# noveens/reviews4rec

Hardware: AMD Instinct MI355X
Metric: train ratings/sec (higher is better)
Workload: dtype f32

## Files before the change

### include/r4r.h

```cpp
#ifndef R4R_H
#define R4R_H

#include <stddef.h>
#include <stdint.h>

#ifdef __cplusplus
extern "C" {
#endif

#define R4R_OK 0
#define R4R_ERR_ARG (-1)
#define R4R_ERR_LAUNCH (-2)
#define R4R_ERR_WORKSPACE (-3)

int r4r_version(void);
const char *r4r_last_error(void);

size_t r4r_textcnn_ws_bytes(int64_t N, int T, int E, int F, int64_t V);
int r4r_textcnn_fwd(const float *table, int64_t V, const int64_t *idx,
                    const float *conv_w, const float *conv_b,
                    float *pooled, int32_t *argmax,
                    void *ws, size_t ws_bytes,
                    int64_t N, int T, int E, int F, void *stream);

// ... 67 lines not shown
int r4r_sqdist_mean_fwd(const float *a, const float *b, float *out, int64_t N, int L, void *stream);
int r4r_sqdist_mean_bwd(const float *a, const float *b, const float *g_out, float *g_a, float *g_b,
                        int64_t N, int L, void *stream);

int r4r_adam_chunk_elems(void);
int r4r_adam_multi(int ntensor, const uint64_t *p, const uint64_t *g, const uint64_t *m, const uint64_t *v,
                   const int64_t *numel, float lr, double beta1, double beta2, float eps,
                   float weight_decay, int64_t step, const int64_t *step_dev, void *stream);
int r4r_adam_gathered(float *p, const float *gathered, int world, float *g_sum, float *m, float *v,
                      int64_t numel, float lr, double beta1, double beta2, float eps,
                      float weight_decay, int64_t step, void *stream);
int r4r_adam_gathered_guarded(float *p, const float *gathered, int world, float *g_sum, float *m, float *v,
                              int64_t numel, float lr, double beta1, double beta2, float eps,
                              float weight_decay, int64_t step, const uint32_t *abort_word, void *stream);

int r4r_peer_segment_create(int64_t bytes, void **ptr, uint8_t *handle);
int r4r_peer_segment_open(const uint8_t *handle, void **ptr);
int r4r_peer_segment_close(void *ptr);
int r4r_peer_segment_destroy(void *ptr);
int r4r_peer_push(const float *src, int64_t numel, const uint64_t *peer_dst, const uint64_t *peer_flags,
                  uint32_t *arrive, int rank, int world, uint32_t epoch, const uint32_t *wait_flags,
                  uint32_t *timed_out, double timeout_s, void *stream);
int r4r_peer_wait(const uint32_t *flags, int world, uint32_t epoch, uint32_t *timed_out, double timeout_s, void *stream);


#define R4R_CONV_AUTO 0
#define R4R_CONV_DIRECT 1
#define R4R_CONV_PROJECT 2
int r4r_deepconn_nparam(void);
int r4r_deepconn_layout(int E, int L, int64_t *offsets, int64_t *sizes, int64_t *total);
size_t r4r_deepconn_ws_bytes(int64_t B, int T, int E, int L, int64_t V);
size_t r4r_deepconn_ws_mult_offset(int64_t B, int T, int E, int L, int64_t V);
size_t r4r_deepconn_ws_count_offset(int64_t B, int T, int E, int L, int64_t V, int tower, int buffer);
int r4r_deepconn_step(const float *table, int64_t V, const int64_t *user_idx, const int64_t *item_idx,
                      const float *y, float *flat_p, float *flat_g,
                      float *pred, float *se, float *sse_accum,
                      void *ws, size_t ws_bytes,
                      int64_t B, int T, int E, int L,
                      float dropout_p, int training, uint64_t seed, uint64_t offset,
                      float inv_denom, int conv_algo, int token_buffer, int tokens_ready,
                      const int64_t *next_user_idx, const int64_t *next_item_idx,
                      float *flat_m, float *flat_v, float lr, double beta1, double beta2, float eps,
                      float weight_decay, int64_t adam_step, void *stream);
int r4r_deepconn_tokens(const int64_t *user_idx, const int64_t *item_idx, void *ws, size_t ws_bytes,
                        int64_t B, int T, int E, int L, int64_t V, int conv_algo, int token_buffer,
                        int discard, void *stream);

#define R4R_TIMING_TEXTCNN_FWD 0
#define R4R_TIMING_TEXTCNN_WGRAD 1
#define R4R_TIMING_ADAM 2
#define R4R_TIMING_PROJ_GEMM 3
#define R4R_TIMING_PROJ_GATHER 4
#define R4R_TIMING_SLOTS 8
int r4r_timing_enable(int slot_mask);
int r4r_timing_read(int slot, double *total_ms, int64_t *count, int reset);

size_t r4r_mf_ws_bytes(int64_t B, int D, int64_t n_users, int64_t n_items);
size_t r4r_mf_ws_persist_bytes(int64_t B, int D, int64_t n_users, int64_t n_items);
size_t r4r_mf_ws_mult_offset(int64_t B, int D, int64_t n_users, int64_t n_items);
size_t r4r_mf_ws_grad_offset(int64_t B, int D, int64_t n_users, int64_t n_items, int which);
int r4r_mf_step(const int64_t *uid, const int64_t *iid, const float *y,
                const uint64_t *p, const uint64_t *m, const uint64_t *v,
                int64_t n_users, int64_t n_items, int D,
                float *pred, float *se, float *sse_accum, void *ws, size_t ws_bytes, int64_t B,
                float dropout_p, int training, uint64_t seed, uint64_t offset, float inv_denom,
                int sweep_period, int64_t sweep_base, int sweep_all,
                float lr, double beta1, double beta2, float eps, float weight_decay, int64_t adam_step,
                void *stream);

int r4r_mf_rows_flush(const uint64_t *p, const uint64_t *m, const uint64_t *v,
                      int64_t n_users, int64_t n_items, int D, void *ws, size_t ws_bytes, int64_t B,
                      int sweep_period, int64_t sweep_base,
                      float lr, double beta1, double beta2, float eps, float weight_decay, int64_t adam_step,
                      void *stream);
size_t r4r_mf_ws_flag_offset(int64_t B, int D, int64_t n_users, int64_t n_items);

// ... 337 lines not shown
```

### reviews4rec_amd/csrc/common.h

```cpp
#pragma once
#include <hip/hip_runtime.h>
#include <hip/hip_ext.h>
#include <stdint.h>
#include <stdio.h>

#include "../../include/r4r.h"

namespace r4r {

void set_error(const char *fmt, ...);

bool timing_on();
void timing_begin(int id, hipStream_t st, void **token);
void timing_begin(int id, hipStream_t st, void **token, bool chain);
void timing_end(void *token, hipStream_t st);

bool timing_kernel_events(int id, hipEvent_t *start, hipEvent_t *stop);

struct ScopedTiming {
    void *tok = nullptr;
    hipStream_t st;
    ScopedTiming(int id, hipStream_t s, bool chain = false) : st(s) { if (timing_on()) timing_begin(id, s, &tok, chain); }
    ~ScopedTiming() { if (tok) timing_end(tok, st); }
};
// ... 55 lines not shown
__device__ __forceinline__ void wave_lds_fence() {
    __builtin_amdgcn_fence(__ATOMIC_RELEASE, "wavefront");
    __builtin_amdgcn_wave_barrier();
    __builtin_amdgcn_fence(__ATOMIC_ACQUIRE, "wavefront");
}

__device__ __forceinline__ uint32_t philox_first_word(uint64_t ctr, uint64_t seed) {
    uint32_t c0 = (uint32_t)ctr, c1 = (uint32_t)(ctr >> 32), c2 = 0u, c3 = 0u;
    uint32_t k0 = (uint32_t)seed, k1 = (uint32_t)(seed >> 32);
#pragma unroll
    for (int r = 0; r < 10; ++r) {
        const uint64_t p0 = (uint64_t)0xD2511F53u * c0;
        const uint64_t p1 = (uint64_t)0xCD9E8D57u * c2;
        const uint32_t n0 = (uint32_t)(p1 >> 32) ^ c1 ^ k0;
        const uint32_t n1 = (uint32_t)p1;
        const uint32_t n2 = (uint32_t)(p0 >> 32) ^ c3 ^ k1;
        const uint32_t n3 = (uint32_t)p0;
        c0 = n0; c1 = n1; c2 = n2; c3 = n3;
        k0 += 0x9E3779B9u; k1 += 0xBB67AE85u;
    }
    return c0;
}

inline int64_t cdiv(int64_t a, int64_t b) { return (a + b - 1) / b; }

template <class T>
__device__ __forceinline__ const T &kernel_args() {
    typedef const T __attribute__((address_space(4))) *kernarg_ptr;
    kernarg_ptr p = (kernarg_ptr)__builtin_amdgcn_kernarg_segment_ptr();
    asm volatile("" : "+s"(p));
    return *(const T *)p;
}


}
```

### reviews4rec_amd/csrc/engine.hip

```cpp
#include <stdlib.h>

#include "trace_device.h"
#include "textcnn.h"
#include "wgrad_device.h"
#include "tokens_device.h"
#include "adam_device.h"

namespace r4r {

constexpr int F_CONV = 100;
constexpr int FM_K = 8;
constexpr int MAX_L = 128;

enum { P_UCW = 0, P_UCB, P_UFW, P_UFB, P_ICW, P_ICB, P_IFW, P_IFB, P_FMV, P_FMLW, P_FMLB, P_GB, P_COUNT };

struct Layout {
    int64_t off[P_COUNT], size[P_COUNT], total;
};

static Layout make_layout(int E, int L) {
    Layout lay;
    const int64_t sz[P_COUNT] = {(int64_t)F_CONV * 3 * E, F_CONV, (int64_t)L * F_CONV, L,
                                 (int64_t)F_CONV * 3 * E, F_CONV, (int64_t)L * F_CONV, L,
                                 (int64_t)2 * L * FM_K, 2 * L, 1, 1};
    int64_t o = 0;
    for (int i = 0; i < P_COUNT; ++i) {
        lay.off[i] = o;
        lay.size[i] = sz[i];
        o += (sz[i] + 31) & ~(int64_t)31;
    }
    lay.total = o;
    return lay;
}

struct HeadArgs {
    const float *pmax[2]; const int *parg[2];
    const float *fc_w[2]; const float *fc_b[2];
    const float *V, *lin_w, *lin_b, *gbias;
    const float *y;
    float *pooled[2]; int *argmax[2];
    float *g_pooled[2];
    float *mult;
    float *x, *s, *g, *gz;
    float *pred, *se;
    int64_t B;
    int L, tiles, training, want_grad;
    float p_drop, inv_denom;
    uint64_t seed, offset;
};


constexpr int HEAD_MAX_TILES = 8;

#define SEL2(arr, s) ((s) ? (arr)[1] : (arr)[0])
HEAD_TRACE_DEFINE(r4r_debug_dc_head_trace)
template <int ML>
__global__ __launch_bounds__(256) void deepconn_head_wg_kernel(HeadArgs a) {
    HEAD_STAMP(0)
    constexpr int N2 = 2 * ML, PARTS = 256 / N2;
    __shared__ float sw[2][ML][F_CONV + 1];
    __shared__ float sfb[N2], slw[N2], sz[N2];
    __shared__ float sV[N2][FM_K];
    __shared__ float sp[2][F_CONV + 4];
    __shared__ float red[N2][PARTS + 1];
    const int tid = threadIdx.x, lane = tid & 63, w = tid >> 6;
    const int64_t b = blockIdx.x;
    const int L = a.L, n = 2 * L;
    const float lin_b0 = a.lin_b[0], gbias0 = a.gbias[0], yb = a.y ? a.y[b] : 0.f;

    constexpr int FQ = F_CONV / 4;
    typedef float hq4 __attribute__((ext_vector_type(4)));
    constexpr int WREGS = (2 * ML * FQ + 255) / 256;
    hq4 wreg[WREGS];
    const int wtot = 2 * L * FQ;
#pragma unroll
    for (int k = 0; k < WREGS; ++k) {
        const int i = min(tid + 256 * k, wtot - 1);
        const int t = i >= L * FQ;
        wreg[k] = *reinterpret_cast<const hq4 *>(SEL2(a.fc_w, t) + 4 * (i - t * L * FQ));
    }
    const int tn = min(tid, n - 1);
    const float fbreg = SEL2(a.fc_b, tn >= L)[tn - (tn >= L ? L : 0)];
    const float lwreg = a.lin_w[tn];
    constexpr int VREGS = (N2 * FM_K + 255) / 256;
    float vreg[VREGS];
#pragma unroll
    for (int k = 0; k < VREGS; ++k) vreg[k] = a.V[min(tid + 256 * k, n * FM_K - 1)];

    {
        const int t = w >> 1, f = lane + 64 * (w & 1), fc = min(f, F_CONV - 1);
// ... 131 lines not shown
                    float sv = 0.f;
#pragma unroll
                    for (int k = 0; k < FM_K; ++k) if (lane == k) sv = sk_keep[k];
                    a.s[b * FM_K + lane] = sv;
                }
                if (lane == 0) a.g[b] = g;
            }
        }
    }
    if (!want) return;
    __syncthreads();
    HEAD_STAMP(3)
    if (tid < 2 * F_CONV) {
        const int t = tid >= F_CONV, f = tid - t * F_CONV;
        float acc = 0.f;
        for (int l = 0; l < L; ++l) acc = fmaf(sz[t * L + l], sw[t][l][f], acc);
        SEL2(a.g_pooled, t)[b * F_CONV + f] = acc;
    }
    HEAD_STAMP(4)
}

struct HeadGradArgs {
    const float *pooled[2];
    const float *x, *s, *g, *gz;
    const float *V;
    const float *se;
    float *g_fc_w[2], *g_fc_b[2], *g_V, *g_lin_w, *g_lin_b, *g_gb;
    float *sse_accum;
    int64_t B;
    int L;
};

constexpr int HG_ROWS = 16, HG_COLS = 16;
__device__ __forceinline__ void head_grad_block(const HeadGradArgs &a, int blk) {
    __shared__ float red[HG_ROWS][HG_COLS];
    const int ox = threadIdx.x & (HG_COLS - 1), rg = threadIdx.x / HG_COLS;
    const int L = a.L, n = 2 * L;
    const int n_fcw = L * F_CONV;
    const int seg[9] = {n_fcw, L, n_fcw, L, n * FM_K, n, 1, 1, 1};
    int o = blk * HG_COLS + ox;
    int which = -1, local = 0, acc_o = o;
#pragma unroll
    for (int k = 0; k < 9; ++k) {
        if (which < 0) {
            if (acc_o < seg[k]) { which = k; local = acc_o; }
            else acc_o -= seg[k];
        }
    }
    float s = 0.f;
    if (which >= 0) {
        const bool is_w = which == 0 || which == 2, is_b = which == 1 || which == 3, is_v = which == 4, is_lw = which == 5;
        const int t = which >> 1;
        const int wl = local / F_CONV, wf = local - wl * F_CONV;
        const int vi = local / FM_K, vk = local - vi * FM_K;
        const float *pa = (is_w || is_b) ? a.gz : (which == 8 ? a.se : a.g);
        const int64_t sa = (is_w || is_b) ? n : 1;
        const int64_t oa = is_w ? t * L + wl : (is_b ? t * L + local : 0);
        const bool useb = is_w || is_v, usec = is_v || is_lw;
        const float *pb = is_w ? a.pooled[t & 1] : (is_v ? a.s : a.g);
        const int64_t sb = is_w ? F_CONV : (is_v ? FM_K : 1), ob = is_w ? wf : (is_v ? vk : 0);
        const float *pc = usec ? a.x : a.g;
        const int64_t sc = usec ? n : 1, oc = is_v ? vi : (is_lw ? local : 0);
        const float cv = is_v ? a.V[local] : 0.f;
        constexpr int HB = 8;
        for (int64_t b0 = rg; b0 < a.B; b0 += (int64_t)HG_ROWS * HB) {
            float va[HB], vb[HB], vc[HB];
#pragma unroll
            for (int k = 0; k < HB; ++k) {
                const int64_t b = min(b0 + (int64_t)k * HG_ROWS, a.B - 1);
                va[k] = pa[b * sa + oa];
                vb[k] = pb[b * sb + ob];
                vc[k] = pc[b * sc + oc];
            }
#pragma unroll
            for (int k = 0; k < HB; ++k) {
                const float B_ = useb ? vb[k] : 1.f, C_ = usec ? vc[k] : 1.f;
                const float term = va[k] * (B_ * C_ - C_ * C_ * cv);
                if (b0 + (int64_t)k * HG_ROWS < a.B) s += term;
            }
        }
    }
    red[rg][ox] = s;
    __syncthreads();
    if (rg == 0 && which >= 0) {
        float t = 0.f;
#pragma unroll
        for (int r = 0; r < HG_ROWS; ++r) t += red[r][ox];
        switch (which) {
            case 0: a.g_fc_w[0][local] = t; break;
            case 1: a.g_fc_b[0][local] = t; break;
            case 2: a.g_fc_w[1][local] = t; break;
            case 3: a.g_fc_b[1][local] = t; break;
            case 4: a.g_V[local] = t; break;
            case 5: a.g_lin_w[local] = t; break;
            case 6: a.g_lin_b[0] = t; break;
            case 7: a.g_gb[0] = t; break;
            default: if (a.sse_accum) a.sse_accum[0] += t; break;
        }
    }
}

BWD_TRACE_DEFINE(r4r_debug_dc_bwd_trace)
struct DcBackwardArgs {
    WgradArgs w;
    HeadGradArgs h;
    int hg_blocks;
    TokenArgs nx;
};
__global__ __launch_bounds__(WG_THREADS, 8) void deepconn_backward_kernel(DcBackwardArgs) {
    const DcBackwardArgs &A = kernel_args<DcBackwardArgs>();
    const WgradArgs &w = A.w;
    const HeadGradArgs &h = A.h;
    const TokenArgs &nx = A.nx;
    const int hg_blocks = A.hg_blocks;
    BWD_STAMP(0, wall_clock64())
    BWD_STAMP(2, (unsigned long long)blockIdx.z + 1)
    if (blockIdx.z == 1 || blockIdx.z == 2) {
        wgrad_block(w, blockIdx.x, blockIdx.y, blockIdx.z - 1);
    } else if (blockIdx.z == 0) {
        for (int blk = blockIdx.y * gridDim.x + blockIdx.x; blk < hg_blocks; blk += gridDim.x * gridDim.y) {
            head_grad_block(h, blk);
            __syncthreads();
        }
    } else {
        token_mark_block(nx, blockIdx.y * gridDim.x + blockIdx.x, gridDim.x * gridDim.y, WG_THREADS);
    }
#ifdef R4R_TRACE
    __syncthreads();
#endif
    BWD_STAMP(1, wall_clock64())
}

constexpr int RED_THREADS = 256;
struct FusedAdam {
    float *p, *m, *v;
    const float *g;
    int64_t lo[2], hi[2];
    AdamScalars s;
    int on;
};
__global__ __launch_bounds__(RED_THREADS) void deepconn_reduce_kernel(WgradArgs w, int red_blocks, int comp_blocks,
                                                                      TokenArgs nx, FusedAdam opt) {
    const int bx = blockIdx.x;
    if (bx < red_blocks) {
        const WgradTower &tw = w.t[blockIdx.y];
        const int nw = w.F * 3 * w.E;
        const int i = bx * RED_THREADS + threadIdx.x;
        const float *gp0 = i < nw ? tw.d_w + i : (i < nw + w.F ? tw.d_b + (i - nw) : nullptr);
        const int64_t o = gp0 ? gp0 - opt.g : 0;
        float P = 0.f, M = 0.f, V = 0.f;
        if (opt.on && gp0) { P = opt.p[o]; M = opt.m[o]; V = opt.v[o]; }
        float *dst;
        const float g = wgrad_reduce_elem(w, blockIdx.y, i, dst);
        if (opt.on && dst) {
            adam_elem(P, g, M, V, opt.s);
            opt.p[o] = P; opt.m[o] = M; opt.v[o] = V;
        }
    } else if (bx < red_blocks + comp_blocks) {
        token_compact_auto<RED_THREADS / 64>(nx.t[blockIdx.y], nx.V, bx - red_blocks);
    } else {
        const int64_t o = opt.lo[blockIdx.y] + (int64_t)(bx - red_blocks - comp_blocks) * RED_THREADS + threadIdx.x;
        if (o < opt.hi[blockIdx.y]) {
            float P = opt.p[o], M = opt.m[o], V = opt.v[o];
            adam_elem(P, opt.g[o], M, V, opt.s);
            opt.p[o] = P; opt.m[o] = M; opt.v[o] = V;
        }
    }
}

__global__ void sse_only_kernel(const float *__restrict__ se, float *__restrict__ accum, int64_t B) {
    __shared__ float red[256];
    float s = 0.f;
    for (int64_t i = threadIdx.x; i < B; i += 256) s += se[i];
    red[threadIdx.x] = s;
    __syncthreads();
    for (int off = 128; off > 0; off >>= 1) {
        if ((int)threadIdx.x < off) red[threadIdx.x] += red[threadIdx.x + off];
        __syncthreads();
    }
    if (threadIdx.x == 0) accum[0] += red[0];
}

struct StepWs {
    float *wp[2], *pmax[2]; int *parg[2];
    int *flags[2][2], *slot[2][2], *list[2][2], *count[2][2]; float *ptab[2];
    float *pooled[2]; int *argmax[2]; float *g_pooled[2];
    float *mult, *x, *s, *g, *gz;
    float *part_w[2], *part_b[2];
    size_t bytes;
};

static StepWs carve(void *ws, int64_t B, int T, int E, int L, int64_t V) {
    StepWs w;
    char *p = static_cast<char *>(ws);
    auto take = [&](size_t nbytes) { char *r = p; p += align256(nbytes); return r; };
    const size_t tiles128 = (size_t)(T + 2 + 127) / 128;
    const int ns = textcnn_wgrad_splits(B);
    for (int t = 0; t < 2; ++t) {
        w.wp[t] = reinterpret_cast<float *>(take(textcnn_wp_floats(E) * 4));
        w.pmax[t] = reinterpret_cast<float *>(take((size_t)B * tiles128 * NP * 4));
        w.parg[t] = reinterpret_cast<int *>(take((size_t)B * tiles128 * NP * 4));
        w.pooled[t] = reinterpret_cast<float *>(take((size_t)B * F_CONV * 4));
// ... 17 lines not shown
    w.bytes = (size_t)(p - static_cast<char *>(ws));
    return w;
}

}

using namespace r4r;

extern "C" int r4r_deepconn_nparam(void) { return P_COUNT; }

extern "C" int r4r_deepconn_layout(int E, int L, int64_t *offsets, int64_t *sizes, int64_t *total) {
    R4R_REQUIRE(E > 0 && L > 0 && L <= MAX_L && offsets && sizes && total, "deepconn_layout: bad arguments");
    const Layout lay = make_layout(E, L);
    for (int i = 0; i < P_COUNT; ++i) { offsets[i] = lay.off[i]; sizes[i] = lay.size[i]; }
    *total = lay.total;
    return R4R_OK;
}

extern "C" size_t r4r_deepconn_ws_bytes(int64_t B, int T, int E, int L, int64_t V) {
    if (B < 0 || T <= 0 || E <= 0 || L <= 0 || V <= 0) return 0;
    return carve(nullptr, B, T, E, L, V).bytes;
}

extern "C" size_t r4r_deepconn_ws_mult_offset(int64_t B, int T, int E, int L, int64_t V) {
    char base[1];
    const StepWs w = carve(base, B, T, E, L, V);
    return (size_t)(reinterpret_cast<char *>(w.mult) - base);
}

extern "C" size_t r4r_deepconn_ws_count_offset(int64_t B, int T, int E, int L, int64_t V, int tower, int buffer) {
    char base[1];
    const StepWs w = carve(base, B, T, E, L, V);
    return (size_t)(reinterpret_cast<char *>(w.count[buffer & 1][tower & 1]) - base);
}

extern "C" int r4r_deepconn_tokens(const int64_t *user_idx, const int64_t *item_idx, void *ws, size_t ws_bytes,
                                   int64_t B, int T, int E, int L, int64_t V, int conv_algo, int token_buffer,
                                   int discard, void *stream) {
    R4R_REQUIRE(user_idx && item_idx && ws, "deepconn_tokens: null pointer");
    R4R_REQUIRE(token_buffer == 0 || token_buffer == 1, "deepconn_tokens: token_buffer must be 0 or 1");
    if (ws_bytes < r4r_deepconn_ws_bytes(B, T, E, L, V)) {
        set_error("deepconn_tokens: workspace %zu < %zu bytes", ws_bytes, r4r_deepconn_ws_bytes(B, T, E, L, V));
        return R4R_ERR_WORKSPACE;
    }
    if (B == 0 || textcnn_pick_algo(conv_algo, B, T, E, F_CONV) != R4R_CONV_PROJECT) return R4R_OK;
    const StepWs w = carve(ws, B, T, E, L, V);
    if (discard) {
        for (int t = 0; t < 2; ++t) (void)hipMemsetAsync(w.count[token_buffer][t], 0, sizeof(int), as_stream(stream));
        return check_launch("deepconn_tokens(discard)");
    }
    ProjTower pt[2];
    const int64_t *idx[2] = {user_idx, item_idx};
    for (int t = 0; t < 2; ++t) {
        pt[t] = ProjTower{};
        pt[t].idx = idx[t];
        pt[t].flags = w.flags[token_buffer][t]; pt[t].slot = w.slot[token_buffer][t];
        pt[t].list = w.list[token_buffer][t]; pt[t].count = w.count[token_buffer][t];
    }
    return textcnn_proj_tokens_launch(V, pt, 2, B, T, false, as_stream(stream));
}

extern "C" int r4r_deepconn_step(const float *table, int64_t V, const int64_t *user_idx, const int64_t *item_idx,
                                 const float *y, float *flat_p, float *flat_g,
                                 float *pred, float *se, float *sse_accum,
                                 void *ws, size_t ws_bytes,
                                 int64_t B, int T, int E, int L,
// ... 43 lines not shown
            pt[t].conv_w = P[t ? P_ICW : P_UCW];
            pt[t].conv_b = P[t ? P_ICB : P_UCB];
            pt[t].flags = w.flags[token_buffer][t]; pt[t].slot = w.slot[token_buffer][t];
            pt[t].list = w.list[token_buffer][t]; pt[t].count = w.count[token_buffer][t];
            pt[t].ptab = w.ptab[t]; pt[t].pmax = w.pmax[t]; pt[t].parg = w.parg[t]; pt[t].wimg = w.wp[t];
        }
        if (!tokens_ready)
            if (int rc = textcnn_proj_tokens_launch(V, pt, 2, B, T, false, st)) return rc;
        if (int rc = textcnn_proj_compute_launch(table, V, pt, 2, B, T, E, F_CONV, st)) return rc;
        tiles = proj_tiles(T);
    } else {
        FwdTower ft[2];
        for (int t = 0; t < 2; ++t) {
            ft[t].idx = idx[t];
            ft[t].conv_w = P[t ? P_ICW : P_UCW];
            ft[t].conv_b = P[t ? P_ICB : P_UCB];
            ft[t].wp = w.wp[t]; ft[t].pmax = w.pmax[t]; ft[t].parg = w.parg[t];
        }
        if (int rc = textcnn_fwd_launch(table, ft, 2, B, T, E, F_CONV, st)) return rc;
        tiles = textcnn_tiles(T);
    }

    HeadArgs h;
    for (int t = 0; t < 2; ++t) {
        h.pmax[t] = w.pmax[t]; h.parg[t] = w.parg[t];
        h.fc_w[t] = P[t ? P_IFW : P_UFW]; h.fc_b[t] = P[t ? P_IFB : P_UFB];
        h.pooled[t] = w.pooled[t]; h.argmax[t] = w.argmax[t]; h.g_pooled[t] = w.g_pooled[t];
    }
    h.V = P[P_FMV]; h.lin_w = P[P_FMLW]; h.lin_b = P[P_FMLB]; h.gbias = P[P_GB];
    h.y = y; h.mult = w.mult; h.x = w.x; h.s = w.s; h.g = w.g; h.gz = w.gz;
    h.pred = pred; h.se = se;
    h.B = B; h.L = L; h.tiles = tiles; h.training = training; h.want_grad = flat_g != nullptr;
    h.p_drop = dropout_p; h.inv_denom = inv_denom; h.seed = seed; h.offset = offset;
    if (L <= 16) deepconn_head_wg_kernel<16><<<(unsigned)B, 256, 0, st>>>(h);
    else if (L <= 32) deepconn_head_wg_kernel<32><<<(unsigned)B, 256, 0, st>>>(h);
    else if (L <= 64) deepconn_head_wg_kernel<64><<<(unsigned)B, 256, 0, st>>>(h);
    else deepconn_head_wg_kernel<128><<<(unsigned)B, 256, 0, st>>>(h);

    if (!flat_g) {
        if (y && sse_accum) sse_only_kernel<<<1, 256, 0, st>>>(se, sse_accum, B);
        return check_launch("deepconn_step(forward)");
    }

    HeadGradArgs hg;
    for (int t = 0; t < 2; ++t) {
        hg.pooled[t] = w.pooled[t];
        hg.g_fc_w[t] = G[t ? P_IFW : P_UFW]; hg.g_fc_b[t] = G[t ? P_IFB : P_UFB];
    }
    hg.x = w.x; hg.s = w.s; hg.g = w.g; hg.gz = w.gz; hg.V = P[P_FMV]; hg.se = se;
    hg.g_V = G[P_FMV]; hg.g_lin_w = G[P_FMLW]; hg.g_lin_b = G[P_FMLB]; hg.g_gb = G[P_GB];
    hg.sse_accum = sse_accum; hg.B = B; hg.L = L;
    const int nout = 2 * (L * F_CONV + L) + 2 * L * FM_K + 2 * L + 3;
    const int hg_blocks = (nout + HG_COLS - 1) / HG_COLS;

    WgradTower wt[2];
    WgradArgs wa;
    for (int t = 0; t < 2; ++t) {
        wt[t].idx = idx[t]; wt[t].g_pooled = w.g_pooled[t]; wt[t].argmax = w.argmax[t];
        wt[t].part_w = w.part_w[t]; wt[t].part_b = w.part_b[t];
        wt[t].d_w = G[t ? P_ICW : P_UCW]; wt[t].d_b = G[t ? P_ICB : P_UCB];
    }
    for (int k = 0; k < MAX_TOWERS; ++k) wa.t[k] = wt[k < 2 ? k : 0];
    wa.table = table; wa.N = B; wa.T = T; wa.E = E; wa.F = F_CONV;
    wa.table_bytes = (int64_t)V * E * 4;
    wa.nsplit = textcnn_wgrad_splits(B);
    wa.per_split = (int)cdiv(B, wa.nsplit);
    const bool prefetch = next_user_idx && algo == R4R_CONV_PROJECT;
    TokenArgs nx{};
    if (prefetch) {
        ProjTower nt[2];
        const int64_t *nidx[2] = {next_user_idx, next_item_idx};
        const int ob = token_buffer ^ 1;
        for (int t = 0; t < 2; ++t) {
            nt[t] = ProjTower{};
            nt[t].idx = nidx[t];
            nt[t].flags = w.flags[ob][t]; nt[t].slot = w.slot[ob][t];
            nt[t].list = w.list[ob][t]; nt[t].count = w.count[ob][t];
        }
        nx = make_token_args(V, nt, 2, B, T);
    }
    {
        ScopedTiming tm(R4R_TIMING_TEXTCNN_WGRAD, st);
        deepconn_backward_kernel<<<dim3(F_CONV, wa.nsplit, prefetch ? 4 : 3), WG_THREADS, 0, st>>>(DcBackwardArgs{wa, hg, hg_blocks, nx});
    }
    const int red_blocks = (F_CONV * 3 * E + F_CONV + RED_THREADS - 1) / RED_THREADS;
    const int comp_blocks = prefetch ? (int)cdiv((V + 3) / 4, RED_THREADS * compact_groups(V)) : 0;
    FusedAdam opt{};
    int opt_blocks = 0;
    if (flat_m) {
        opt.on = 1;
        opt.p = flat_p; opt.m = flat_m; opt.v = flat_v; opt.g = flat_g;
        opt.lo[0] = lay.off[P_UFW]; opt.hi[0] = lay.off[P_ICW];
        opt.lo[1] = lay.off[P_IFW]; opt.hi[1] = lay.total;
        opt.s = adam_make_scalars(lr, beta1, beta2, eps, weight_decay, adam_step, nullptr);
        const int64_t longest = opt.hi[0] - opt.lo[0] > opt.hi[1] - opt.lo[1] ? opt.hi[0] - opt.lo[0] : opt.hi[1] - opt.lo[1];
        opt_blocks = (int)cdiv(longest, RED_THREADS);
    }
    deepconn_reduce_kernel<<<dim3(red_blocks + comp_blocks + opt_blocks, 2), RED_THREADS, 0, st>>>(
        wa, red_blocks, comp_blocks, nx, opt);
    return check_launch("deepconn_step");
}

extern "C" int r4r_sse_accumulate(const float *se, int64_t n, float *accum, void *stream) {
    R4R_REQUIRE(accum && (se || n == 0) && n >= 0, "sse_accumulate: bad arguments");
    if (n == 0) return R4R_OK;
    sse_only_kernel<<<1, 256, 0, as_stream(stream)>>>(se, accum, n);
    return check_launch("sse_accumulate");
}
```

### reviews4rec_amd/csrc/wgrad_device.h

```cpp
#pragma once
#include "textcnn.h"

namespace r4r {

typedef float wg_f32x4 __attribute__((ext_vector_type(4)));

constexpr int WG_THREADS = 256;

struct WgradArgs {
    WgradTower t[MAX_TOWERS];
    const float *table;
    int64_t N;
    int T, E, F, per_split, nsplit;
    int64_t table_bytes = 0;
};

constexpr int WG_CHUNK = 16;
constexpr int WG_FLIGHT = 8;

template <bool FIRST>
__device__ __forceinline__ void wgrad_block_pass(const WgradArgs &a, int f, int s, int tower, int v0,
                                                 long (&s_off)[WG_CHUNK][3], float (&s_g)[WG_CHUNK]) {
    const WgradTower &tw = a.t[tower];
    const float *__restrict__ table = a.table;
    const int64_t *__restrict__ idx = tw.idx;
    const float *__restrict__ gp = tw.g_pooled;
    const int *__restrict__ argmax = tw.argmax;
    const int T = a.T, E = a.E, F = a.F;
    const int64_t n0 = (int64_t)s * a.per_split;
    const int64_t n1 = min(a.N, n0 + (int64_t)a.per_split);
    const int nvec = 3 * E / 4;
    const int tid = threadIdx.x;
    wg_f32x4 acc[2] = {(wg_f32x4){0.f, 0.f, 0.f, 0.f}, (wg_f32x4){0.f, 0.f, 0.f, 0.f}};
    int vj[2], ve[2];
#pragma unroll
    for (int k = 0; k < 2; ++k) {
        const int v = v0 + tid + k * WG_THREADS;
        vj[k] = (v * 4) / E;
        ve[k] = v * 4 - vj[k] * E;
    }
    float sb = 0.f;
    const bool buf_ok = a.table_bytes > 0 && a.table_bytes < (1ll << 32);
    const __amdgpu_buffer_rsrc_t rsrc = __builtin_amdgcn_make_buffer_rsrc(const_cast<float *>(table), 0, buf_ok ? (int)(unsigned)a.table_bytes : 0, 0x00020000);
    for (int64_t c0 = n0; c0 < n1; c0 += WG_CHUNK) {
        const int nd = (int)min((int64_t)WG_CHUNK, n1 - c0);
        __syncthreads();
        if (tid < nd * 3) {
            const int d = tid / 3, j = tid - d * 3;
            const int64_t n = c0 + d;
            const int p = argmax[n * F + f];
// ... 28 lines not shown
                        }
                    }
                }
            }
        } else {
#pragma unroll
            for (int k = 0; k < 2; ++k) {
                if (v0 + tid + k * WG_THREADS < nvec) {
#pragma unroll 4
                    for (int d = 0; d < nd; ++d) {
                        const long off = s_off[d][vj[k]];
                        if (off >= 0) acc[k] += s_g[d] * *reinterpret_cast<const wg_f32x4 *>(table + off + ve[k]);
                    }
                }
            }
        }
        if (FIRST && tid == 0)
            for (int d = 0; d < nd; ++d) sb += s_g[d];
    }
#pragma unroll
    for (int k = 0; k < 2; ++k) {
        const int v = v0 + tid + k * WG_THREADS;
        if (v < nvec) *reinterpret_cast<wg_f32x4 *>(tw.part_w + ((size_t)s * F + f) * 3 * E + v * 4) = acc[k];
    }
    if (FIRST && tid == 0) tw.part_b[(size_t)s * F + f] = sb;
}

__device__ __forceinline__ void wgrad_block(const WgradArgs &a, int f, int s, int tower) {
    __shared__ long s_off[WG_CHUNK][3];
    __shared__ float s_g[WG_CHUNK];
    wgrad_block_pass<true>(a, f, s, tower, 0, s_off, s_g);
    const int nvec = 3 * a.E / 4;
    for (int v0 = 2 * WG_THREADS; v0 < nvec; v0 += 2 * WG_THREADS) wgrad_block_pass<false>(a, f, s, tower, v0, s_off, s_g);
}


constexpr int WG_SUPER = 96;
static_assert(WG_SUPER % WG_CHUNK == 0, "whole streaming rounds per resolved super-chunk");
__device__ __forceinline__ void wgrad_block_packed(const WgradArgs &a, int fgroup, int s, int tower) {
    __shared__ long p_off[4][WG_SUPER][3];
    __shared__ float p_g[4][WG_SUPER];
    const WgradTower &tw = a.t[tower];
    const float *__restrict__ table = a.table;
    const int64_t *__restrict__ idx = tw.idx;
    const float *__restrict__ gp = tw.g_pooled;
    const int *__restrict__ argmax = tw.argmax;
    const int T = a.T, E = a.E, F = a.F;
    const int64_t n0 = (int64_t)s * a.per_split;
    const int64_t n1 = min(a.N, n0 + (int64_t)a.per_split);
    const int nvec = 3 * E / 4;
    const int wave = threadIdx.x >> 6, lane = threadIdx.x & 63;
    const int f = fgroup * 4 + wave;
    const bool live = f < F;
    wg_f32x4 acc = (wg_f32x4){0.f, 0.f, 0.f, 0.f};
    const int vj = (lane * 4) / E, ve = lane * 4 - vj * E;
    float sb = 0.f;
    constexpr int NRES = (WG_SUPER * 3 + 63) / 64;
    for (int64_t c0 = n0; c0 < n1; c0 += WG_SUPER) {
        const int nd = (int)min((int64_t)WG_SUPER, n1 - c0);
        __syncthreads();
        if (live) {
            int pv[NRES];
            float gv[NRES];
#pragma unroll
            for (int k = 0; k < NRES; ++k) {
                const int i = lane + 64 * k, d = i / 3;
// ... 18 lines not shown
            for (int k = 0; k < NRES; ++k) off[k] = onv[k] ? tokv[k] * E : -1;
#pragma unroll
            for (int k = 0; k < NRES; ++k) {
                const int i = lane + 64 * k, d = i / 3, j = i - d * 3;
                if (d < WG_SUPER) {
                    p_off[wave][d][j] = off[k];
                    if (j == 0) p_g[wave][d] = pv[k] >= 0 ? gv[k] : 0.f;
                }
            }
        }
        __syncthreads();
        if (live && lane < nvec) {
            for (int r0 = 0; r0 < nd; r0 += WG_CHUNK) {
                wg_f32x4 v[WG_CHUNK];
#pragma unroll
                for (int d = 0; d < WG_CHUNK; ++d) {
                    const long off = p_off[wave][r0 + d][vj];
                    v[d] = *reinterpret_cast<const wg_f32x4 *>(table + (off < 0 ? 0 : off) + ve);
                }
#pragma unroll
                for (int d = 0; d < WG_CHUNK; ++d) {
                    const wg_f32x4 sum = acc + p_g[wave][r0 + d] * v[d];
                    acc = p_off[wave][r0 + d][vj] >= 0 ? sum : acc;
                }
            }
        }
        if (live && lane == 0)
            for (int d = 0; d < nd; ++d) sb += p_g[wave][d];
    }
    if (live && lane < nvec) *reinterpret_cast<wg_f32x4 *>(tw.part_w + ((size_t)s * F + f) * 3 * E + lane * 4) = acc;
    if (live && lane == 0) tw.part_b[(size_t)s * F + f] = sb;
}

constexpr int WG_MAX_SPLITS = 16;

__device__ __forceinline__ float wgrad_reduce_elem(const WgradArgs &a, int tower, int i, float *&dst) {
    const WgradTower &tw = a.t[tower];
    const int nw = a.F * 3 * a.E;
    const float *src;
    size_t stride;
    if (i < nw) { src = tw.part_w + i; stride = (size_t)nw; dst = tw.d_w + i; }
    else if (i < nw + a.F) { src = tw.part_b + (i - nw); stride = (size_t)a.F; dst = tw.d_b + (i - nw); }
    else { dst = nullptr; return 0.f; }
    float v[WG_MAX_SPLITS];
#pragma unroll
    for (int k = 0; k < WG_MAX_SPLITS; ++k) v[k] = src[(size_t)(k < a.nsplit ? k : 0) * stride];
    float s = 0.f;
#pragma unroll
    for (int k = 0; k < WG_MAX_SPLITS; ++k)
        if (k < a.nsplit) s += v[k];
    *dst = s;
    return s;
}

__device__ __forceinline__ void wgrad_reduce_block(const WgradArgs &a, int tower, int blk) {
    float *dst;
    (void)wgrad_reduce_elem(a, tower, blk * (int)blockDim.x + (int)threadIdx.x, dst);
}

}
```

Before: 1.389 million.

## Fuse DeepCoNN conv wgrad, split reduction and Adam into one owned-row backward kernel

Adds an 'owned' backward path where each workgroup owns one conv weight row (filter, tap, tower). It accumulates all batch splits in LDS, reduces them, and applies Adam in place, so the separate partial-sum, reduce and optimizer launches for those parameters go away. Head-gradient blocks also apply Adam inline, and token compaction for the next batch is folded into the same grid. Token-mark blocks are appended to the forward head kernel, read through a second kernarg struct. Fewer launches and no partial buffers in global memory, at the cost of large 1024-thread blocks, buffer-resource loads limited to tables under 4GB, and more complex launch geometry.

Result: faster. 1.414 million (median of 5 runs) (+1.8%).

```diff
diff --git a/include/r4r.h b/include/r4r.h
--- a/include/r4r.h
+++ b/include/r4r.h
@@ -123,6 +123,7 @@
 size_t r4r_deepconn_ws_bytes(int64_t B, int T, int E, int L, int64_t V);
 size_t r4r_deepconn_ws_mult_offset(int64_t B, int T, int E, int L, int64_t V);
 size_t r4r_deepconn_ws_count_offset(int64_t B, int T, int E, int L, int64_t V, int tower, int buffer);
+size_t r4r_deepconn_ws_token_offset(int64_t B, int T, int E, int L, int64_t V, int tower, int buffer, int what);
 int r4r_deepconn_step(const float *table, int64_t V, const int64_t *user_idx, const int64_t *item_idx,
                       const float *y, float *flat_p, float *flat_g,
                       float *pred, float *se, float *sse_accum,
@@ -133,6 +134,7 @@
                       const int64_t *next_user_idx, const int64_t *next_item_idx,
                       float *flat_m, float *flat_v, float lr, double beta1, double beta2, float eps,
                       float weight_decay, int64_t adam_step, void *stream);
+int r4r_deepconn_wgrad_owned(int64_t B, int E, int64_t V, int fused_opt);
 int r4r_deepconn_tokens(const int64_t *user_idx, const int64_t *item_idx, void *ws, size_t ws_bytes,
                         int64_t B, int T, int E, int L, int64_t V, int conv_algo, int token_buffer,
                         int discard, void *stream);
diff --git a/reviews4rec_amd/csrc/common.h b/reviews4rec_amd/csrc/common.h
--- a/reviews4rec_amd/csrc/common.h
+++ b/reviews4rec_amd/csrc/common.h
@@ -111,5 +111,12 @@
     return *(const T *)p;
 }
 
+template <class T>
+__device__ __forceinline__ const T &kernel_args_at(size_t offset) {
+    typedef const char __attribute__((address_space(4))) *kernarg_ptr;
+    kernarg_ptr p = (kernarg_ptr)__builtin_amdgcn_kernarg_segment_ptr();
+    asm volatile("" : "+s"(p));
+    return *(const T *)(p + offset);
+}
 
 }
diff --git a/reviews4rec_amd/csrc/engine.hip b/reviews4rec_amd/csrc/engine.hip
--- a/reviews4rec_amd/csrc/engine.hip
+++ b/reviews4rec_amd/csrc/engine.hip
@@ -53,9 +53,19 @@
 constexpr int HEAD_MAX_TILES = 8;
 
 #define SEL2(arr, s) ((s) ? (arr)[1] : (arr)[0])
+struct HeadMarkArgs {
+    TokenArgs nx;
+    int blocks;
+};
+static_assert(sizeof(HeadArgs) % alignof(HeadMarkArgs) == 0, "the second kernel parameter starts where the first ends");
 HEAD_TRACE_DEFINE(r4r_debug_dc_head_trace)
 template <int ML>
-__global__ __launch_bounds__(256) void deepconn_head_wg_kernel(HeadArgs a) {
+__global__ __launch_bounds__(256) void deepconn_head_wg_kernel(HeadArgs a, HeadMarkArgs) {
+    if ((int64_t)blockIdx.x >= a.B) {
+        const HeadMarkArgs &mk = kernel_args_at<HeadMarkArgs>(sizeof(HeadArgs));
+        token_mark_block(mk.nx, (int)(blockIdx.x - (unsigned)a.B), mk.blocks, 256);
+        return;
+    }
     HEAD_STAMP(0)
     constexpr int N2 = 2 * ML, PARTS = 256 / N2;
     __shared__ float sw[2][ML][F_CONV + 1];
@@ -253,7 +263,8 @@
 };
 
 constexpr int HG_ROWS = 16, HG_COLS = 16;
-__device__ __forceinline__ void head_grad_block(const HeadGradArgs &a, int blk) {
+template <bool ADAM>
+__device__ __forceinline__ void head_grad_block(const HeadGradArgs &a, int blk, const WgradAdam *opt) {
     __shared__ float red[HG_ROWS][HG_COLS];
     const int ox = threadIdx.x & (HG_COLS - 1), rg = threadIdx.x / HG_COLS;
     const int L = a.L, n = 2 * L;
@@ -301,12 +312,31 @@
             }
         }
     }
+    float *dst = nullptr;
+    int64_t od = 0;
+    float P = 0.f, M = 0.f, V = 0.f;
+    if (ADAM && rg == 0 && which >= 0 && which < 8) {
+        dst = which == 0 ? a.g_fc_w[0] : (which == 1 ? a.g_fc_b[0] : (which == 2 ? a.g_fc_w[1] : (which == 3 ? a.g_fc_b[1] :
+              (which == 4 ? a.g_V : (which == 5 ? a.g_lin_w : (which == 6 ? a.g_lin_b : a.g_gb))))));
+        dst += local;
+        od = dst - opt->g;
+        P = opt->p[od]; M = opt->m[od]; V = opt->v[od];
+    }
     red[rg][ox] = s;
     __syncthreads();
     if (rg == 0 && which >= 0) {
         float t = 0.f;
 #pragma unroll
         for (int r = 0; r < HG_ROWS; ++r) t += red[r][ox];
+        if constexpr (ADAM) {
+            if (dst) {
+                *dst = t;
+                adam_elem(P, t, M, V, opt->s);
+                opt->p[od] = P; opt->m[od] = M; opt->v[od] = V;
+            } else if (a.sse_accum) {
+                a.sse_accum[0] += t;
+            }
+        } else {
         switch (which) {
             case 0: a.g_fc_w[0][local] = t; break;
             case 1: a.g_fc_b[0][local] = t; break;
@@ -317,6 +347,7 @@
             case 6: a.g_lin_b[0] = t; break;
             case 7: a.g_gb[0] = t; break;
             default: if (a.sse_accum) a.sse_accum[0] += t; break;
+        }
         }
     }
 }
@@ -340,7 +371,7 @@
         wgrad_block(w, blockIdx.x, blockIdx.y, blockIdx.z - 1);
     } else if (blockIdx.z == 0) {
         for (int blk = blockIdx.y * gridDim.x + blockIdx.x; blk < hg_blocks; blk += gridDim.x * gridDim.y) {
-            head_grad_block(h, blk);
+            head_grad_block<false>(h, blk, nullptr);
             __syncthreads();
         }
     } else {
@@ -389,6 +420,41 @@
     }
 }
 
+constexpr int OWNED_COMPACT_BIG_G = 4;
+struct DcOwnedArgs {
+    WgradArgs w;
+    HeadGradArgs h;
+    int hg_blocks, comp_blocks;
+    TokenArgs nx;
+    WgradAdam opt;
+};
+__global__ __launch_bounds__(WG_OWNED_MAX_THREADS, 8) void deepconn_backward_owned_kernel(DcOwnedArgs) {
+    extern __shared__ wg_f32x4 s_part[];
+    const DcOwnedArgs &A = kernel_args<DcOwnedArgs>();
+    const int bx = blockIdx.x, hg_blocks = A.hg_blocks;
+    constexpr int ROWS = 2 * F_CONV * 3;
+    if (bx >= hg_blocks && bx < hg_blocks + ROWS) {
+        const int r = bx - hg_blocks, tower = r / (F_CONV * 3), fj = r - tower * (F_CONV * 3), f = fj / 3;
+        wgrad_owned_block(A.w, A.opt, f, fj - f * 3, tower, s_part);
+        return;
+    }
+    if (threadIdx.x >= 256) return;
+    if (bx < hg_blocks) {
+        head_grad_block<true>(A.h, bx, &A.opt);
+    } else {
+        const int c = bx - hg_blocks - ROWS, comp_blocks = A.comp_blocks, tower = c >= comp_blocks;
+        if (A.nx.V > COMPACT_BIG_V) token_compact_block<4, OWNED_COMPACT_BIG_G>(A.nx.t[tower], A.nx.V, c - tower * comp_blocks);
+        else token_compact_block<4, 1>(A.nx.t[tower], A.nx.V, c - tower * comp_blocks);
+    }
+}
+
+static bool deepconn_owned(int64_t B, int E, int64_t V, bool fused_opt) {
+    if (!fused_opt || B <= 0) return false;
+    if (!wgrad_owned_fits(E, textcnn_wgrad_splits(B), V * (int64_t)E * 4)) return false;
+    const char *e = getenv("R4R_WGRAD_OWNED");
+    return !(e && e[0] == '0');
+}
+
 __global__ void sse_only_kernel(const float *__restrict__ se, float *__restrict__ accum, int64_t B) {
     __shared__ float red[256];
     float s = 0.f;
@@ -472,6 +538,17 @@
     char base[1];
     const StepWs w = carve(base, B, T, E, L, V);
     return (size_t)(reinterpret_cast<char *>(w.count[buffer & 1][tower & 1]) - base);
+}
+
+extern "C" int r4r_deepconn_wgrad_owned(int64_t B, int E, int64_t V, int fused_opt) {
+    return deepconn_owned(B, E, V, fused_opt != 0) ? 1 : 0;
+}
+
+extern "C" size_t r4r_deepconn_ws_token_offset(int64_t B, int T, int E, int L, int64_t V, int tower, int buffer, int what) {
+    char base[1];
+    const StepWs w = carve(base, B, T, E, L, V);
+    const int *p = what ? w.list[buffer & 1][tower & 1] : w.slot[buffer & 1][tower & 1];
+    return (size_t)(reinterpret_cast<const char *>(p) - base);
 }
 
 extern "C" int r4r_deepconn_tokens(const int64_t *user_idx, const int64_t *item_idx, void *ws, size_t ws_bytes,
@@ -581,40 +658,8 @@
     h.pred = pred; h.se = se;
     h.B = B; h.L = L; h.tiles = tiles; h.training = training; h.want_grad = flat_g != nullptr;
     h.p_drop = dropout_p; h.inv_denom = inv_denom; h.seed = seed; h.offset = offset;
-    if (L <= 16) deepconn_head_wg_kernel<16><<<(unsigned)B, 256, 0, st>>>(h);
-    else if (L <= 32) deepconn_head_wg_kernel<32><<<(unsigned)B, 256, 0, st>>>(h);
-    else if (L <= 64) deepconn_head_wg_kernel<64><<<(unsigned)B, 256, 0, st>>>(h);
-    else deepconn_head_wg_kernel<128><<<(unsigned)B, 256, 0, st>>>(h);
-
-    if (!flat_g) {
-        if (y && sse_accum) sse_only_kernel<<<1, 256, 0, st>>>(se, sse_accum, B);
-        return check_launch("deepconn_step(forward)");
-    }
-
-    HeadGradArgs hg;
-    for (int t = 0; t < 2; ++t) {
-        hg.pooled[t] = w.pooled[t];
-        hg.g_fc_w[t] = G[t ? P_IFW : P_UFW]; hg.g_fc_b[t] = G[t ? P_IFB : P_UFB];
-    }
-    hg.x = w.x; hg.s = w.s; hg.g = w.g; hg.gz = w.gz; hg.V = P[P_FMV]; hg.se = se;
-    hg.g_V = G[P_FMV]; hg.g_lin_w = G[P_FMLW]; hg.g_lin_b = G[P_FMLB]; hg.g_gb = G[P_GB];
-    hg.sse_accum = sse_accum; hg.B = B; hg.L = L;
-    const int nout = 2 * (L * F_CONV + L) + 2 * L * FM_K + 2 * L + 3;
-    const int hg_blocks = (nout + HG_COLS - 1) / HG_COLS;
-
-    WgradTower wt[2];
-    WgradArgs wa;
-    for (int t = 0; t < 2; ++t) {
-        wt[t].idx = idx[t]; wt[t].g_pooled = w.g_pooled[t]; wt[t].argmax = w.argmax[t];
-        wt[t].part_w = w.part_w[t]; wt[t].part_b = w.part_b[t];
-        wt[t].d_w = G[t ? P_ICW : P_UCW]; wt[t].d_b = G[t ? P_ICB : P_UCB];
-    }
-    for (int k = 0; k < MAX_TOWERS; ++k) wa.t[k] = wt[k < 2 ? k : 0];
-    wa.table = table; wa.N = B; wa.T = T; wa.E = E; wa.F = F_CONV;
-    wa.table_bytes = (int64_t)V * E * 4;
-    wa.nsplit = textcnn_wgrad_splits(B);
-    wa.per_split = (int)cdiv(B, wa.nsplit);
-    const bool prefetch = next_user_idx && algo == R4R_CONV_PROJECT;
+    const bool prefetch = flat_g && next_user_idx && algo == R4R_CONV_PROJECT;
+    const bool owned = flat_g && deepconn_owned(B, E, V, flat_m != nullptr);
     TokenArgs nx{};
     if (prefetch) {
         ProjTower nt[2];
@@ -628,12 +673,59 @@
         }
         nx = make_token_args(V, nt, 2, B, T);
     }
+    HeadMarkArgs mk{nx, 0};
+    if (owned && prefetch) mk.blocks = (int)(cdiv(B * (int64_t)T, 256) < 1024 ? cdiv(B * (int64_t)T, 256) : 1024);
+    const unsigned head_wgs = (unsigned)B + (unsigned)mk.blocks;
+    if (L <= 16) deepconn_head_wg_kernel<16><<<head_wgs, 256, 0, st>>>(h, mk);
+    else if (L <= 32) deepconn_head_wg_kernel<32><<<head_wgs, 256, 0, st>>>(h, mk);
+    else if (L <= 64) deepconn_head_wg_kernel<64><<<head_wgs, 256, 0, st>>>(h, mk);
+    else deepconn_head_wg_kernel<128><<<head_wgs, 256, 0, st>>>(h, mk);
+
+    if (!flat_g) {
+        if (y && sse_accum) sse_only_kernel<<<1, 256, 0, st>>>(se, sse_accum, B);
+        return check_launch("deepconn_step(forward)");
+    }
+
+    HeadGradArgs hg;
+    for (int t = 0; t < 2; ++t) {
+        hg.pooled[t] = w.pooled[t];
+        hg.g_fc_w[t] = G[t ? P_IFW : P_UFW]; hg.g_fc_b[t] = G[t ? P_IFB : P_UFB];
+    }
+    hg.x = w.x; hg.s = w.s; hg.g = w.g; hg.gz = w.gz; hg.V = P[P_FMV]; hg.se = se;
+    hg.g_V = G[P_FMV]; hg.g_lin_w = G[P_FMLW]; hg.g_lin_b = G[P_FMLB]; hg.g_gb = G[P_GB];
+    hg.sse_accum = sse_accum; hg.B = B; hg.L = L;
+    const int nout = 2 * (L * F_CONV + L) + 2 * L * FM_K + 2 * L + 3;
+    const int hg_blocks = (nout + HG_COLS - 1) / HG_COLS;
+
+    WgradTower wt[2];
+    WgradArgs wa;
+    for (int t = 0; t < 2; ++t) {
+        wt[t].idx = idx[t]; wt[t].g_pooled = w.g_pooled[t]; wt[t].argmax = w.argmax[t];
+        wt[t].part_w = w.part_w[t]; wt[t].part_b = w.part_b[t];
+        wt[t].d_w = G[t ? P_ICW : P_UCW]; wt[t].d_b = G[t ? P_ICB : P_UCB];
+    }
+    for (int k = 0; k < MAX_TOWERS; ++k) wa.t[k] = wt[k < 2 ? k : 0];
+    wa.table = table; wa.N = B; wa.T = T; wa.E = E; wa.F = F_CONV;
+    wa.table_bytes = (int64_t)V * E * 4;
+    wa.nsplit = textcnn_wgrad_splits(B);
+    wa.per_split = (int)cdiv(B, wa.nsplit);
+    const int comp_g = owned ? (V > COMPACT_BIG_V ? OWNED_COMPACT_BIG_G : 1) : compact_groups(V);
+    const int comp_blocks = prefetch ? (int)cdiv((V + 3) / 4, RED_THREADS * comp_g) : 0;
+    if (owned) {
+        DcOwnedArgs oa{wa, hg, hg_blocks, comp_blocks, nx, WgradAdam{}};
+        oa.opt.p = flat_p; oa.opt.m = flat_m; oa.opt.v = flat_v; oa.opt.g = flat_g;
+        oa.opt.s = adam_make_scalars(lr, beta1, beta2, eps, weight_decay, adam_step, nullptr);
+        const int threads = wgrad_owned_threads(E, wa.nsplit);
+        ScopedTiming tm(R4R_TIMING_TEXTCNN_WGRAD, st);
+        deepconn_backward_owned_kernel<<<dim3((unsigned)(hg_blocks + 2 * F_CONV * 3 + 2 * comp_blocks)), threads,
+                                         (size_t)threads * sizeof(wg_f32x4), st>>>(oa);
+        return check_launch("deepconn_step");
+    }
     {
         ScopedTiming tm(R4R_TIMING_TEXTCNN_WGRAD, st);
         deepconn_backward_kernel<<<dim3(F_CONV, wa.nsplit, prefetch ? 4 : 3), WG_THREADS, 0, st>>>(DcBackwardArgs{wa, hg, hg_blocks, nx});
     }
     const int red_blocks = (F_CONV * 3 * E + F_CONV + RED_THREADS - 1) / RED_THREADS;
-    const int comp_blocks = prefetch ? (int)cdiv((V + 3) / 4, RED_THREADS * compact_groups(V)) : 0;
     FusedAdam opt{};
     int opt_blocks = 0;
     if (flat_m) {
diff --git a/reviews4rec_amd/csrc/wgrad_device.h b/reviews4rec_amd/csrc/wgrad_device.h
--- a/reviews4rec_amd/csrc/wgrad_device.h
+++ b/reviews4rec_amd/csrc/wgrad_device.h
@@ -1,5 +1,6 @@
 #pragma once
 #include "textcnn.h"
+#include "adam_device.h"
 
 namespace r4r {
 
@@ -16,6 +17,7 @@
 };
 
 constexpr int WG_CHUNK = 16;
+constexpr int WG_MAX_SPLITS = 16;
 constexpr int WG_FLIGHT = 8;
 
 template <bool FIRST>
@@ -110,6 +112,123 @@
     wgrad_block_pass<true>(a, f, s, tower, 0, s_off, s_g);
     const int nvec = 3 * a.E / 4;
     for (int v0 = 2 * WG_THREADS; v0 < nvec; v0 += 2 * WG_THREADS) wgrad_block_pass<false>(a, f, s, tower, v0, s_off, s_g);
+}
+
+
+constexpr int WG_OWNED_MAX_THREADS = 1024;
+
+struct WgradAdam {
+    float *p, *m, *v;
+    const float *g;
+    AdamScalars s;
+};
+
+static inline bool wgrad_owned_fits(int E, int nsplit, int64_t table_bytes) {
+    return E > 85 && E <= 680 && E % 4 == 0 && nsplit <= WG_MAX_SPLITS && nsplit * (E / 4) <= WG_OWNED_MAX_THREADS &&
+           table_bytes > 0 && table_bytes < (1ll << 32);
+}
+static inline int wgrad_owned_threads(int E, int nsplit) {
+    const int n = (nsplit * (E / 4) + 63) & ~63;
+    return n < WG_THREADS ? WG_THREADS : n;
+}
+
+__device__ __forceinline__ void wgrad_owned_block(const WgradArgs &a, const WgradAdam &opt, int f, int j, int tower,
+                                                  wg_f32x4 *s_part) {
+    __shared__ unsigned s_bo[WG_MAX_SPLITS][WG_CHUNK];
+    __shared__ float s_g[WG_MAX_SPLITS][WG_CHUNK];
+    __shared__ float s_pb[WG_MAX_SPLITS];
+    const WgradTower &tw = a.t[tower];
+    const int64_t *__restrict__ idx = tw.idx;
+    const float *__restrict__ gp = tw.g_pooled;
+    const int *__restrict__ argmax = tw.argmax;
+    const int T = a.T, E = a.E, F = a.F, nsplit = a.nsplit, per_split = a.per_split;
+    const int nq = E >> 2;
+    const int tid = threadIdx.x;
+    const int s = tid / nq, q = tid - s * nq;
+    const bool live = s < nsplit;
+    const bool bias = j == 0 && tid == 0;
+
+    float *const gw = tw.d_w + ((size_t)f * 3 + j) * E + q * 4;
+    const int64_t ow = gw - opt.g, ob = (tw.d_b + f) - opt.g;
+    wg_f32x4 P = (wg_f32x4){0.f, 0.f, 0.f, 0.f}, M = P, V = P;
+    float Pb = 0.f, Mb = 0.f, Vb = 0.f;
+
+    const __amdgpu_buffer_rsrc_t rsrc = __builtin_amdgcn_make_buffer_rsrc(const_cast<float *>(a.table), 0, (int)(unsigned)a.table_bytes, 0x00020000);
+    const int n0 = s * per_split, n1 = min((int)a.N, n0 + per_split);
+    wg_f32x4 acc = (wg_f32x4){0.f, 0.f, 0.f, 0.f};
+    float sb = 0.f;
+    for (int c = 0; c < per_split; c += WG_CHUNK) {
+        __syncthreads();
+        if (tid < nsplit * WG_CHUNK) {
+            const int rs = tid / WG_CHUNK, d = tid - rs * WG_CHUNK;
+            const int64_t n = (int64_t)rs * per_split + c + d;
+            unsigned bo = ~0u;
+            float gv = 0.f;
+            if (c + d < per_split && n < a.N) {
+                const int p = argmax[n * F + f];
+                const float g = gp[n * F + f];
+                const int t = p - 2 + j;
+                if (p >= 0 && t >= 0 && t < T) bo = (unsigned)((uint64_t)idx[n * T + t] * (uint64_t)E * 4u);
+                gv = (p >= 0) ? g : 0.f;
+            }
+            s_bo[rs][d] = bo;
+            s_g[rs][d] = gv;
+        }
+        __syncthreads();
+        if (live) {
+#pragma unroll
+            for (int d0 = 0; d0 < WG_CHUNK; d0 += WG_FLIGHT) {
+                wg_f32x4 row[WG_FLIGHT];
+                bool on[WG_FLIGHT];
+#pragma unroll
+                for (int u = 0; u < WG_FLIGHT; ++u) {
+                    const unsigned bo = s_bo[s][d0 + u];
+                    on[u] = bo != ~0u;
+                    row[u] = __builtin_bit_cast(wg_f32x4, __builtin_amdgcn_raw_buffer_load_b128(rsrc, (int)(on[u] ? bo + (unsigned)q * 16u : 0xfffffff0u), 0, 0));
+                }
+#pragma unroll
+                for (int u = 0; u < WG_FLIGHT; ++u) {
+                    const wg_f32x4 sum = acc + s_g[s][d0 + u] * row[u];
+                    acc = on[u] ? sum : acc;
+                }
+                __builtin_amdgcn_sched_barrier(0);
+            }
+            if (j == 0 && q == 0) {
+                const int nd = max(0, min(WG_CHUNK, n1 - (n0 + c)));
+                for (int d = 0; d < nd; ++d) sb += s_g[s][d];
+            }
+        }
+    }
+    if (s == 0) {
+        P = *reinterpret_cast<const wg_f32x4 *>(opt.p + ow);
+        M = *reinterpret_cast<const wg_f32x4 *>(opt.m + ow);
+        V = *reinterpret_cast<const wg_f32x4 *>(opt.v + ow);
+    }
+    if (bias) { Pb = opt.p[ob]; Mb = opt.m[ob]; Vb = opt.v[ob]; }
+    s_part[tid] = acc;
+    if (live && j == 0 && q == 0) s_pb[s] = sb;
+    __syncthreads();
+    if (s == 0) {
+        wg_f32x4 g = (wg_f32x4){0.f, 0.f, 0.f, 0.f};
+        for (int k = 0; k < nsplit; ++k) g += s_part[k * nq + q];
+        *reinterpret_cast<wg_f32x4 *>(gw) = g;
+#pragma unroll
+        for (int e = 0; e < 4; ++e) {
+            float pe = P[e], me = M[e], ve = V[e];
+            adam_elem(pe, g[e], me, ve, opt.s);
+            P[e] = pe; M[e] = me; V[e] = ve;
+        }
+        *reinterpret_cast<wg_f32x4 *>(opt.p + ow) = P;
+        *reinterpret_cast<wg_f32x4 *>(opt.m + ow) = M;
+        *reinterpret_cast<wg_f32x4 *>(opt.v + ow) = V;
+    }
+    if (bias) {
+        float g = 0.f;
+        for (int k = 0; k < nsplit; ++k) g += s_pb[k];
+        tw.d_b[f] = g;
+        adam_elem(Pb, g, Mb, Vb, opt.s);
+        opt.p[ob] = Pb; opt.m[ob] = Mb; opt.v[ob] = Vb;
+    }
 }
 
 
@@ -194,7 +313,6 @@
     if (live && lane == 0) tw.part_b[(size_t)s * F + f] = sb;
 }
 
-constexpr int WG_MAX_SPLITS = 16;
 
 __device__ __forceinline__ float wgrad_reduce_elem(const WgradArgs &a, int tower, int i, float *&dst) {
     const WgradTower &tw = a.t[tower];
```
